# USTC-StarTeam/DR4SR

Measured on AMD Instinct MI355X. Metric: training sequences/sec, SASRec d=64 L=50, higher is better.
Workload: dtype f32; 1 GPU; SASRec on amazon-toys-shaped synthetic rows (BASELINE configs[1]): N=11925, L=50, d=64, 2 layers, 2 heads, FFN 128, dropout 0.50, B=256 rows/GPU/step, toys histogram (10.9% valid) seqlen; global_batch=256, seq_len=50, parallelism=dp1, hip_graph=True, steps_per_graph=30

## Files before the change

### dr4sr_amd/csrc/kernels.h

```cpp
#pragma once
#include <hip/hip_runtime.h>
#include <stdint.h>
#include "../../include/dr4sr_hip.h"
#include "../../include/dr4sr_hip_hooks.h"
#include "prep_body.h"

#define DR4SR_MAX_LAYERS 8

struct LayerWs {
    float* qkv;
    float* ctx;
    float* attn_st;
    unsigned* attn_keep;
    float* u1;
    float* y;
    float* st1;
    float* a;
    float* h;
    float* u2;
    float* st2;
    float* df;
    float* da;
    float* du1;
    float* dout;
// ... 73 lines not shown
    float* rd; int n_head;
    float* ln_part;
    const int* state; uint64_t seed; float p; float eps; int layer; int training;
    uint32_t sP, sA, sF;
    unsigned long long* stamps;
    const float* nx_in_w; const float* nx_in_b; float* nx_qkv;
    const float* up_dqkv; const float* up_in_w; const float* up_du1;
    const float* up_kv_part;
    TileAttnArgs at;
    int xcd;
    float* nx_dqkv_zero;
    float* dn_dqkv_zero;
    int wt_attn;
    unsigned short* row_keep;
    const unsigned short* sp;
};

struct EmbQkvArgs {
    const float* E; const float* P; const int64_t* idx; const int64_t* rows; const int* cu; const int* tile_seq; float* X;
    const float* W; const float* bias; float* QKV; const int* state;
    int B, L, n_items, training; uint64_t seed; float p;
    int* idx32;
    int2* tok; float* dqkv_zero;
    int xcd;
    int wf_layers;
    const unsigned short* sp;
    const float* inw;
};
struct QkvEmbBwdArgs {
    const float* dQKV; const float* W; const float* dU1; const int64_t* idx; const int64_t* rows; const int* cu; const int* tile_seq;
    float* dE; float* dP; const int* state; int B, L, n_items, training; uint64_t seed; float p;
    float* gout;
    const float* kv_part; const int2* tok;
    const unsigned short* sp;
    const float* inw; float* d_inw; const float* E; const float* P;
#ifdef DR4SR_EXPERIMENTS
    int xskip;
#endif
};

struct ScoreTileArgs {
    const float* E; float* dE; const int64_t* target; const int64_t* rows; const int* cu; const int* tile_seq; int64_t* neg_item; float* part;
    int sample_neg, n_items, B, L;
    int4* rec;
    int4* ent; unsigned char* off; const int* idx32; int logG;
    const float* phi; const float* gumbel; const int64_t* user_id; const unsigned long long* gate_in; unsigned long long* gate_out;
    float* w_out; float inv_tau; uint64_t meta_seed;
};

struct WgradJob {
    const float* G; int ldg; int gcol;
    const float* X; int ldx;
    float* dW; float* db;
    int ldw;
};
#define DR4SR_DET_MAX_SPLITS 320
#define DR4SR_WGRAD_MAX_JOBS 12
struct WgradArgs {
    WgradJob job[DR4SR_WGRAD_MAX_JOBS * DR4SR_MAX_LAYERS];
    int jobs_per_layer;
    const int* state; uint64_t seed; float p; int training;
    const float* ln_part; int64_t ln_layer_stride; float* grads; int64_t o_ln1_w; int64_t layer_stride;
    const float* score_part; float* tail; int B; int D;
    int score_tiles;
    int ln_tile_rows;
    int ln_rows[DR4SR_MAX_LAYERS];
    int qeb_plane;
    int layer0;
    int bf16x3;
    int xcd;
// ... 26 lines not shown
int carve_workspace(const dr4sr_sasrec_plan* p, Workspace* ws);

int launch_prep(const dr4sr_sasrec_plan* p, const Workspace& ws, int bump_rng, int zero_grads, hipStream_t s, int adam_bc = 0);
int make_prep_args(const dr4sr_sasrec_plan* p, const Workspace& ws, int bump_rng, PrepArgs* out);
int launch_embed_fwd(const dr4sr_sasrec_plan* p, const Workspace& ws, int training, hipStream_t s, const float* inw = nullptr);
int launch_embed_bwd(const dr4sr_sasrec_plan* p, const Workspace& ws, int training, hipStream_t s, const float* inw = nullptr, float* d_inw = nullptr);
int launch_unpack(const dr4sr_sasrec_plan* p, const Workspace& ws, const float* X, float* out, int mode, hipStream_t s);
int launch_pack(const dr4sr_sasrec_plan* p, const Workspace& ws, const float* dout, float* dX, int mode, hipStream_t s);

int launch_transpose_weights(const dr4sr_sasrec_plan* p, const Workspace& ws, hipStream_t s);
bool tile_bf3(const dr4sr_sasrec_plan* p, const Workspace& ws);
int launch_wsplit(const dr4sr_sasrec_plan* p, const Workspace& ws, hipStream_t s);
int launch_wfrag_write(const dr4sr_sasrec_plan* p, const Workspace& ws, hipStream_t s);
bool wfrag_img_on(const dr4sr_sasrec_plan* p, const Workspace& ws);
int launch_wsplit_raw(const float* params, unsigned short* img, int64_t o_in, int64_t o_out, int64_t o_w1, int64_t o_w2, int64_t layer_stride,
                      int E, int D, int F, int n_layer, hipStream_t s);
int launch_embqkv_fwd(const dr4sr_sasrec_plan* p, const Workspace& ws, int training, hipStream_t s, const float* inw = nullptr);
int launch_qkv_embed_bwd(const dr4sr_sasrec_plan* p, const Workspace& ws, int training, hipStream_t s, const float* inw = nullptr, float* d_inw = nullptr);
int launch_post_mid(const dr4sr_sasrec_plan* p, const Workspace& ws, int training, hipStream_t s, const dr4sr_meta_weighting* mw = nullptr);
int launch_qkv_fwd(const dr4sr_sasrec_plan* p, const Workspace& ws, int layer, hipStream_t s);
int launch_post_fwd(const dr4sr_sasrec_plan* p, const Workspace& ws, int layer, int training, hipStream_t s);
int launch_post_bwd(const dr4sr_sasrec_plan* p, const Workspace& ws, int layer, int training, hipStream_t s);
int launch_qkv_bwd(const dr4sr_sasrec_plan* p, const Workspace& ws, int layer, hipStream_t s);
int launch_wgrad(const dr4sr_sasrec_plan* p, const Workspace& ws, int training, int with_score, hipStream_t s, bool qeb = false,
                 bool meta = false, int l_lo = 0, int l_hi = -1, int table = -1, const float* inw = nullptr, float* d_inw = nullptr);
bool wgrad_table_jobs(const dr4sr_sasrec_plan* p, const Workspace& ws);
bool attn_in_tile(const dr4sr_sasrec_plan* p, const Workspace& ws);
bool attn_wave_on(const dr4sr_sasrec_plan* p, const Workspace& ws);
bool attn_fold_fwd(const dr4sr_sasrec_plan* p, const Workspace& ws);
PostArgs make_post_args(const dr4sr_sasrec_plan* p, const Workspace& ws, int layer, int training);
int launch_attn_tile_fwd(const dr4sr_sasrec_plan* p, const Workspace& ws, int layer, int training, hipStream_t s);
int launch_attn_tile_bwd(const dr4sr_sasrec_plan* p, const Workspace& ws, int layer, int training, hipStream_t s);
bool qeb_in_wgrad(const Workspace& ws);

int launch_attn_fwd(const dr4sr_sasrec_plan* p, const Workspace& ws, int layer, int training, hipStream_t s);
int launch_attn_bwd(const dr4sr_sasrec_plan* p, const Workspace& ws, int layer, int training, hipStream_t s);

struct GruWaveArgs {
    const float* gi1; const float* whh[2]; const float* wih2; const int* cu;
    float* r[2]; float* z[2]; float* n[2]; float* ghn[2]; float* hprev[2]; float* hout[2];
    const float* dhout; float* dgi[2]; float* dgh[2];
};
int launch_prep_raw(const int64_t* seqlen, const int64_t* rows, int* cu, int* state, int B, int L, int bump_rng, float* zero,
                    int64_t zero_floats, hipStream_t s);
int launch_prep_raw_hints(const int64_t* seqlen, const int64_t* rows, int* cu, int* state, int B, int L, int bump_rng, float* zero,
                          int64_t zero_floats, int* tile_seq, const PermSel& sel, hipStream_t s);
int launch_embed_fwd_raw(const float* E, const float* P, const int64_t* idx, const int64_t* rows, const int* cu, float* X, int B,
                         int L, int D, int n_items, const int* state, uint64_t seed, float p, int training, hipStream_t s, const float* inw = nullptr);
int launch_embed_bwd_raw(const float* dX, const int64_t* idx, const int64_t* rows, const int* cu, float* dE, float* dP, int B, int L,
                         int D, int n_items, const int* state, uint64_t seed, float p, int training, hipStream_t s,
                         const float* inw = nullptr, float* d_inw = nullptr, const float* E = nullptr, const float* P = nullptr);
int launch_unpack_raw(const float* X, const int* cu, float* out, int B, int L, int D, int last, hipStream_t s);
int launch_pack_raw(const float* dout, const int* cu, float* dX, int B, int L, int D, int last, hipStream_t s);
int launch_score_packed_raw(const float* Z, const float* E, float* dE, float* dZ, const int64_t* target, const int64_t* rows,
                            const int* cu, int64_t* neg_item, int sample_neg, float* part, const int* state, uint64_t seed,
                            int n_items, int B, int L, int D, hipStream_t s, int4* rec = nullptr);

int launch_attn2_fwd(const dr4sr_sasrec_plan* p, const Workspace& ws, int layer, int training, hipStream_t s);
int launch_attn2_bwd(const dr4sr_sasrec_plan* p, const Workspace& ws, int layer, int training, hipStream_t s);

int launch_score_packed(const dr4sr_sasrec_plan* p, const Workspace& ws, hipStream_t s);
int launch_adam(const dr4sr_sasrec_plan* p, hipStream_t s, const PrepArgs* next = nullptr);
```

### dr4sr_amd/csrc/linear.hip

```cpp
#include "common.h"
#include "kernels.h"
#include <cstdlib>
#define STAMP(i) do { if (A.stamps && blockIdx.x == 0 && threadIdx.x == 0) A.stamps[i] = __builtin_amdgcn_s_memtime(); } while (0)

extern __shared__ __attribute__((aligned(16))) float smem[];

__global__ __launch_bounds__(256) void k_transpose(const float* __restrict__ params, float* __restrict__ wT,
                                                   int64_t o_in, int64_t o_out, int64_t o_w1, int64_t o_w2,
                                                   int64_t layer_stride, int64_t wT_stride, int D, int F) {
    const int m = blockIdx.y, layer = blockIdx.z;
    const float* src;
    float* dst = wT + layer * wT_stride;
    int R, C;
    if (m == 0) { src = params + o_in + layer * layer_stride; R = 3 * D; C = D; }
    else if (m == 1) { src = params + o_out + layer * layer_stride; R = D; C = D; dst += 3 * D * D; }
    else if (m == 2) { src = params + o_w1 + layer * layer_stride; R = F; C = D; dst += 4 * D * D; }
    else { src = params + o_w2 + layer * layer_stride; R = D; C = F; dst += 4 * D * D + D * F; }
    for (int i = blockIdx.x * 256 + threadIdx.x; i < R * C; i += gridDim.x * 256) {
        const int r = i / C, c = i % C;
        dst[c * R + r] = src[i];
    }
}

int launch_transpose_weights(const dr4sr_sasrec_plan* p, const Workspace& ws, hipStream_t s) {
// ... 216 lines not shown
                o = ld4(A.E + id * D + c);
                const float4 pe = ld4(A.P + (size_t)pos * D + c);
                o = make_float4(o.x + pe.x, o.y + pe.y, o.z + pe.z, o.w + pe.w);
                if constexpr (WGT) {
                    const float w = A.inw[(size_t)b * A.L + pos];
                    o.x *= w; o.y *= w; o.z *= w; o.w *= w;
                }
                if (dodrop) {
                    const float4 m = drop4(rk, DR4SR_SITE_EMB, ((uint64_t)b * A.L + pos) * D + c);
                    o.x *= m.x; o.y *= m.y; o.z *= m.z; o.w *= m.w;
                }
                st4(A.X + (size_t)t * D + c, o);
            }
            st4(As + r * LDA + c, o);
        }
    }
    lds_barrier();
    TileAcc<BM, N> acc;
    tile_zero(acc);
    if constexpr (PFE) tile_mma_frag<BM, D, N>(As, LDA, f_in, acc);
    else tile_gemm<D == 128 && BM == 32, BM, D, N>(As, LDA, A.W, D, false, A.sp, WSplitGeo<D, 128>::E, 0, acc);
    if constexpr (EPB) tile_to_global<BM, N>(acc, A.QKV, N, in_b, t0, T); else tile_to_global<BM, N>(acc, A.QKV, N, A.bias, t0, T);
    if (A.dqkv_zero) zero_kv_rows<BM, D>(A.dqkv_zero, t0, T);
}

int launch_embqkv_fwd(const dr4sr_sasrec_plan* p, const Workspace& ws, int training, hipStream_t s, const float* inw) {
    const int D = p->D, bm = tile_rows(ws);
    const size_t lds = sizeof(float) * bm * (D + 4);
    dim3 grid((ws.Tmax + bm - 1) / bm), blk(256);
    EmbQkvArgs A;
    A.E = p->params + ws.off[0]; A.P = p->params + ws.off[1]; A.idx = p->in_item_id; A.rows = p->rows; A.cu = ws.cu; A.tile_seq = ws.tile_seq; A.X = ws.X[0];
    A.W = p->params + poff(ws, 0, P_IN_W); A.bias = p->params + poff(ws, 0, P_IN_B); A.QKV = ws.layer[0].qkv; A.state = p->state;
    A.B = p->B; A.L = p->L; A.n_items = p->n_items; A.training = training; A.seed = p->seed; A.p = p->p_drop;
    A.idx32 = de_owner_mode(ws) ? ws.idx32 : nullptr;
    A.sp = wsplit_of(p, ws, 0); A.wf_layers = 0; A.inw = inw;
    if (wfrag_img_on(p, ws)) { A.sp = reinterpret_cast<const unsigned short*>(ws.wfrag); A.wf_layers = p->n_layer; }
    const bool in_tile = attn_in_tile(p, ws);
    A.tok = (in_tile || ws.attn_tile_sa || attn_wave_on(p, ws)) ? ws.tok : nullptr; A.dqkv_zero = in_tile ? ws.layer[0].dqkv : nullptr;
    A.xcd = tile_xcd_order(p, ws) ? 1 : 0;
    if (A.xcd) grid.x = xcd_grid((int)grid.x, bm);
    if (wave_tiles(p, ws)) return launch_wt_embqkv_fwd(A, ws.Tmax, s);
#define EQ(B_) do { if (inw) { if (D == 64) hipLaunchKernelGGL((k_embqkv_fwd<B_, 64, true>), grid, blk, lds, s, A); \
                                else hipLaunchKernelGGL((k_embqkv_fwd<B_, 128, true>), grid, blk, lds, s, A); } \
                    else if (D == 64) hipLaunchKernelGGL((k_embqkv_fwd<B_, 64>), grid, blk, lds, s, A); \
                    else hipLaunchKernelGGL((k_embqkv_fwd<B_, 128>), grid, blk, lds, s, A); } while (0)
    BM_DISPATCH(bm, EQ);
#undef EQ
    return DR4SR_LAUNCH_CHECK();
}


struct LnCarry { float4 v; float mean, rstd; uint32_t keep; };
template <int F>
struct RowCarry { LnCarry ln1, ln2; float4 a[F / 64]; uint32_t akeep; };
__host__ __device__ constexpr bool carry_vals(int CARRY) { return CARRY != 0; }
__host__ __device__ constexpr bool carry_bits(int CARRY) { return CARRY == 1 || CARRY == 3; }
__device__ __forceinline__ uint32_t keep_bits4(const float4& m) {
    return (m.x != 0.f ? 1u : 0u) | (m.y != 0.f ? 2u : 0u) | (m.z != 0.f ? 4u : 0u) | (m.w != 0.f ? 8u : 0u);
}
__device__ __forceinline__ float4 keep_factors4(const RngKey& k, uint32_t bits) {
    return make_float4((bits & 1u) ? k.scale : 0.f, (bits & 2u) ? k.scale : 0.f, (bits & 4u) ? k.scale : 0.f, (bits & 8u) ? k.scale : 0.f);
}

template <int BM, int D, bool RES_IN_LDS, bool COPY_LDS, bool CARRY = false, bool KPRE = false, bool NOST = false, bool GPRE = false>
__device__ __forceinline__ void ln_rowpass(const float* __restrict__ Cs, int ldc, const float* res, int ldres,
                                           const float* __restrict__ lnw, const float* __restrict__ lnb, float eps,
                                           float* __restrict__ U, float* __restrict__ OUT, float* __restrict__ ST,
// ... 1244 lines not shown
    tile_zero(acc);
    tile_mma_xw<BM, K, D>(As, LDA, WT, D, acc);
    tile_to_lds<BM, D>(acc, Cs, LDC, nullptr);
    lds_barrier();
    constexpr int C4 = D / 4;
    for (int i = threadIdx.x; i < BM * C4; i += 256) {
        const int row = i / C4, c = (i % C4) * 4;
        if (t0 + row < T) {
            const float4 v = ld4(Cs + row * LDC + c), r = ld4(dU1 + (size_t)(t0 + row) * D + c);
            st4(dXo + (size_t)(t0 + row) * D + c, make_float4(v.x + r.x, v.y + r.y, v.z + r.z, v.w + r.w));
        }
    }
}

int launch_qkv_bwd(const dr4sr_sasrec_plan* p, const Workspace& ws, int layer, hipStream_t s) {
    const int D = p->D, bm = tile_rows(ws);
    const size_t lds = sizeof(float) * bm * ((3 * D + 4) + (D + 4));
    dim3 grid((ws.Tmax + bm - 1) / bm), blk(256);
    const float* WT = p->params + poff(ws, layer, P_IN_W);
    const LayerWs& lw = ws.layer[layer];
#define QB(B_) do { if (D == 64) { big_lds(k_qkv_bwd<B_, 64>, lds); hipLaunchKernelGGL((k_qkv_bwd<B_, 64>), grid, blk, lds, s, lw.dqkv, WT, lw.du1, ws.dX[layer], p->state); } \
                    else { big_lds(k_qkv_bwd<B_, 128>, lds); hipLaunchKernelGGL((k_qkv_bwd<B_, 128>), grid, blk, lds, s, lw.dqkv, WT, lw.du1, ws.dX[layer], p->state); } } while (0)
    BM_DISPATCH(bm, QB);
#undef QB
    return DR4SR_LAUNCH_CHECK();
}


#ifdef DR4SR_EMB_ADDS_FLOAT4
constexpr bool EMB_ADD_ROWS = false;
#else
constexpr bool EMB_ADD_ROWS = true;
#endif
template <int BM, int D, bool DET = false, bool WGT = false>
__device__ __forceinline__ void qkv_embed_bwd_body(const QkvEmbBwdArgs& A, const int t0, const int T) {
    constexpr int K = 3 * D, LDA = K + 4, LDC = D + 4, LPT = D / 4, TPB = 256 / LPT;
    float* As = smem;
    float* Cs = As + BM * LDA;
    float* accP = Cs + BM * LDC;
    int* ids = reinterpret_cast<int*>(accP + A.L * D);
    constexpr bool PFQ = BM == 16 && D == 64;
    WFragC<PFQ ? K : 16, 64> f_in;
    if constexpr (PFQ) wfrag_load(f_in, A.W, D);
    for (int i = threadIdx.x; i < A.L * D; i += 256) accP[i] = 0.f;
    load_tile_bm<BM, K>(As, LDA, A.dQKV, K, t0, T);
    lds_barrier();
    if constexpr (BM == 16 && DET) {
        det_kv_rows<D>(As, LDA, const_cast<float*>(A.dQKV), A.kv_part, A.tok, t0, T);
        lds_barrier();
    }
    TileAcc<BM, D> acc;
    tile_zero(acc);
    if constexpr (PFQ) tile_mma_frag<BM, K, D>(As, LDA, f_in, acc);
    else tile_gemm<D == 128 && BM == 32, BM, K, D>(As, LDA, A.W, D, true, A.sp, WSplitGeo<D, 128>::E, 0, acc);
    tile_to_lds<BM, D>(acc, Cs, LDC, nullptr);
    lds_barrier();
    const int c = (threadIdx.x % LPT) * 4;
    const bool dodrop = A.training && A.p > 0.f;
    const RngKey rk = make_rng(A.seed, (uint32_t)A.state[DR4SR_STATE_RNGSTEP], A.p);
    const int bh = A.tile_seq[t0 >> 4];
#pragma unroll
    for (int r0 = 0; r0 < BM; r0 += TPB) {
        const int r = r0 + threadIdx.x / LPT, t = t0 + r;
        if (r < BM && t < T) {
            const int b = find_seq_from(A.cu, A.B, t, bh), pos = t - A.cu[b];
            const int64_t row = A.rows ? A.rows[b] : b;
            const float4 v = ld4(Cs + r * LDC + c), u = ld4(A.dU1 + (size_t)t * D + c);
            float4 g = make_float4(v.x + u.x, v.y + u.y, v.z + u.z, v.w + u.w);
            if (dodrop) {
                const float4 m = drop4(rk, DR4SR_SITE_EMB, ((uint64_t)b * A.L + pos) * D + c);
                g.x *= m.x; g.y *= m.y; g.z *= m.z; g.w *= m.w;
            }
            if constexpr (WGT) {
                if (A.d_inw) {
                    int64_t ic = A.idx[row * A.L + pos];
                    ic = ic < 0 ? 0 : (ic >= A.n_items ? A.n_items - 1 : ic);
                    const float4 e = ld4(A.E + ic * D + c), pe = ld4(A.P + (size_t)pos * D + c);
                    const float sum = lane_group_sum<LPT>((g.x * (e.x + pe.x) + g.y * (e.y + pe.y)) + (g.z * (e.z + pe.z) + g.w * (e.w + pe.w)));
                    if (c == 0) A.d_inw[(size_t)b * A.L + pos] = sum;
                }
                const float w = A.inw[(size_t)b * A.L + pos];
                g.x *= w; g.y *= w; g.z *= w; g.w *= w;
            }
            if (A.gout) { st4(A.gout + (size_t)t * D + c, g); continue; }
            float* a = accP + pos * D + c;
            atomicAdd(a, g.x); atomicAdd(a + 1, g.y); atomicAdd(a + 2, g.z); atomicAdd(a + 3, g.w);
            const int64_t id = A.idx[row * A.L + pos];
            st4(Cs + r * LDC + c, g);
            if (c == 0) ids[r] = (id > 0 && id < A.n_items) ? (int)id : 0;
        } else if (r < BM && c == 0 && !A.gout) ids[r] = 0;
    }
    if (A.gout) return;
    __syncthreads();
#pragma unroll
    for (int r0 = 0; r0 < BM; r0 += TPB) {
        const int r = r0 + threadIdx.x / LPT;
        const int id = r < BM ? ids[r] : 0;
        unsigned long long same = 0;
        if constexpr (BM <= LPT) {
            const int j = threadIdx.x % LPT;
            const unsigned long long bal = __ballot(j < BM && id > 0 && ids[j < BM ? j : 0] == id);
            same = (bal >> ((threadIdx.x & 63) / LPT * LPT)) & ((1ull << BM) - 1ull);
        } else if (id > 0) {
            for (int q = 0; q < BM; ++q) same |= (unsigned long long)(ids[q] == id) << q;
        }
        if (id > 0 && (same & ((1ull << r) - 1ull)) == 0) {
            if constexpr (!DET && BM == 16 && EMB_ADD_ROWS) {
                const int j = threadIdx.x % LPT;
                float gk[4];
#pragma unroll
                for (int k = 0; k < 4; ++k) gk[k] = Cs[r * LDC + LPT * k + j];
                for (same = r + 1 < 64 ? same >> (r + 1) : 0; same; same &= same - 1) {
                    const int q = r + __ffsll((long long)same);
#pragma unroll
                    for (int k = 0; k < 4; ++k) gk[k] += Cs[q * LDC + LPT * k + j];
                }
                float* d = A.dE + (size_t)id * D + j;
                if (!XSKIP_EMB(A)) {
#pragma unroll
                    for (int k = 0; k < 4; ++k) unsafeAtomicAdd(d + LPT * k, gk[k]);
                }
                continue;
            }
            float4 g = ld4(Cs + r * LDC + c);
            for (same = r + 1 < 64 ? same >> (r + 1) : 0; same; same &= same - 1) {
                const int q = r + __ffsll((long long)same);
                const float4 o = ld4(Cs + q * LDC + c); g.x += o.x; g.y += o.y; g.z += o.z; g.w += o.w;
            }
            float* d = A.dE + (size_t)id * D + c;
            if (!XSKIP_EMB(A)) { unsafeAtomicAdd(d, g.x); unsafeAtomicAdd(d + 1, g.y); unsafeAtomicAdd(d + 2, g.z); unsafeAtomicAdd(d + 3, g.w); }
        }
    }
    for (int i = threadIdx.x; i < A.L * D; i += 256) {
        const float v = accP[i];
        if (v != 0.f) unsafeAtomicAdd(A.dP + i, v);
    }
}
template <int BM, int D, bool DET = false, bool WGT = false>
__global__ __launch_bounds__(256) void k_qkv_embed_bwd(const QkvEmbBwdArgs A) {
    const int T = A.state[DR4SR_STATE_T], t0 = blockIdx.x * BM;
    if (t0 >= T) return;
    qkv_embed_bwd_body<BM, D, DET, WGT>(A, t0, T);
}

static QkvEmbBwdArgs make_qeb_args(const dr4sr_sasrec_plan* p, const Workspace& ws, int training, const float* inw = nullptr, float* d_inw = nullptr) {
    const LayerWs& lw = ws.layer[0];
    QkvEmbBwdArgs A;
    A.dQKV = lw.dqkv; A.W = p->params + poff(ws, 0, P_IN_W); A.dU1 = lw.du1; A.idx = p->in_item_id; A.rows = p->rows; A.cu = ws.cu; A.tile_seq = ws.tile_seq;
    A.dE = p->grads + ws.off[0]; A.dP = p->grads + ws.off[1]; A.state = p->state; A.B = p->B; A.L = p->L; A.n_items = p->n_items;
    A.training = training; A.seed = p->seed; A.p = p->p_drop;
    A.gout = scatter_in_wgrad(ws) ? ws.dX[0] : nullptr;
    A.kv_part = (ws.det_lat && ws.det_kv && attn_in_tile(p, ws)) ? ws.det_kv : nullptr; A.tok = ws.tok;
    A.sp = wsplit_of(p, ws, 0);
    A.inw = inw; A.d_inw = inw ? d_inw : nullptr; A.E = p->params + ws.off[0]; A.P = p->params + ws.off[1];
#ifdef DR4SR_EXPERIMENTS
    A.xskip = DR4SR_XENV("DR4SR_ROWADDS_SKIP") ? (atoi(DR4SR_XENV("DR4SR_ROWADDS_SKIP")) & 4) : 0;
#endif
    return A;
}
bool qeb_in_wgrad(const Workspace& ws) {
    const bool off = DR4SR_ENV("DR4SR_QEB_SEPARATE") != nullptr || DR4SR_ENV("DR4SR_NO_FUSE") != nullptr;
    return !off && tile_rows(ws) == 16 && !ws.det_lat;
}

int launch_qkv_embed_bwd(const dr4sr_sasrec_plan* p, const Workspace& ws, int training, hipStream_t s, const float* inw, float* d_inw) {
    const int D = p->D, bm = tile_rows(ws);
    const size_t lds = sizeof(float) * (bm * ((3 * D + 4) + (D + 4)) + (size_t)p->L * D + bm);
    dim3 grid((ws.Tmax + bm - 1) / bm), blk(256);
    const QkvEmbBwdArgs A = make_qeb_args(p, ws, training, inw, d_inw);
    if (wave_tiles(p, ws) && wt_bwd_on() && A.gout) return launch_wt_qkv_embed_bwd(A, ws.Tmax, s);
#define QEW(B_, D_, DET_) do { big_lds((k_qkv_embed_bwd<B_, D_, DET_, true>), lds); hipLaunchKernelGGL((k_qkv_embed_bwd<B_, D_, DET_, true>), grid, blk, lds, s, A); } while (0)
#define QE(B_) do { if (A.inw) { if (B_ == 16 && A.kv_part) { if (D == 64) QEW(16, 64, true); else QEW(16, 128, true); } \
                                 else if (D == 64) QEW(B_, 64, false); else QEW(B_, 128, false); } \
                    else if (B_ == 16 && A.kv_part) { if (D == 64) { big_lds((k_qkv_embed_bwd<16, 64, true>), lds); hipLaunchKernelGGL((k_qkv_embed_bwd<16, 64, true>), grid, blk, lds, s, A); } \
                                                 else { big_lds((k_qkv_embed_bwd<16, 128, true>), lds); hipLaunchKernelGGL((k_qkv_embed_bwd<16, 128, true>), grid, blk, lds, s, A); } } \
                    else if (D == 64) { big_lds(k_qkv_embed_bwd<B_, 64>, lds); hipLaunchKernelGGL((k_qkv_embed_bwd<B_, 64>), grid, blk, lds, s, A); } \
                    else { big_lds(k_qkv_embed_bwd<B_, 128>, lds); hipLaunchKernelGGL((k_qkv_embed_bwd<B_, 128>), grid, blk, lds, s, A); } } while (0)
    BM_DISPATCH(bm, QE);
#undef QE
#undef QEW
    return DR4SR_LAUNCH_CHECK();
}


#ifdef DR4SR_EXPERIMENTS
#define WGRAD_ADD(P_, V_) do { if (!noadd) unsafeAtomicAdd(P_, V_); } while (0)
#else
#define WGRAD_ADD(P_, V_) unsafeAtomicAdd(P_, V_)
#endif

template <int NG, int KX>
__device__ __forceinline__ void wgrad_body(const WgradJob& J, const WgradArgs& A, float* __restrict__ part = nullptr, const int noadd = 0) {
    constexpr int NT = NG / 32, KT = KX / 32, TPW = (NT * KT) / 4;
    static_assert((NT * KT) % 4 == 0, "tile count must split over 4 waves");
    const int T = A.state[DR4SR_STATE_T];
// ... 379 lines not shown
        qn = 0;
    };
    constexpr int CH = 4;
    for (int base = ia; base < ib; base += 64 * CH) {
        int lo[CH], hi[CH];
#pragma unroll
        for (int k = 0; k < CH; ++k) {
            const int i = base + 64 * k + lane;
            lo[k] = 0; hi[k] = 0;
            if (i < ib) { const unsigned char* o = A.ow_off + (size_t)i * OS + owner; lo[k] = o[0]; hi[k] = o[1]; }
        }
#pragma unroll
        for (int k = 0; k < CH; ++k) {
            unsigned long long m = __ballot(hi[k] > lo[k]);
            while (m) {
                const int L = __ffsll((long long)m) - 1; m &= m - 1;
                const int tile = base + 64 * k + L, e0 = __builtin_amdgcn_readlane(lo[k], L), e1 = __builtin_amdgcn_readlane(hi[k], L);
                for (int e = e0; e < e1; ++e) {
                    if (lane == qn) pend = A.ow_ent[(size_t)tile * E + e];
                    if (++qn == QN) flush();
                }
            }
        }
    }
    flush();
    __syncthreads();
    for (int i = threadIdx.x; i < rpo * D; i += 256) {
        const float sum = (smem[i] + smem[(size_t)rpo * D + i]) + (smem[(size_t)2 * rpo * D + i] + smem[(size_t)3 * rpo * D + i]);
        const int id = ((i / D) << A.ow_logG) | owner;
        if (sum != 0.f && id < A.sc_n_items) A.sc_dE[(size_t)id * D + (i % D)] += sum;
    }
}

template <int D, int F, bool BF, bool SUB = false, bool BLK = false, int TB = 0, bool WGT = false>
__device__ __forceinline__ void wgrad_kernel_body(const WgradArgs& A, const QkvEmbBwdArgs& Q, const int noadd = 0) {
    const int layer = A.layer0 + (A.qeb_plane ? (int)blockIdx.z - 1 : (int)blockIdx.z);
    if (!SUB && layer < A.layer0) {
        const int T = A.state[DR4SR_STATE_T], nblk = gridDim.x * gridDim.y;
        for (int tile = blockIdx.y * gridDim.x + blockIdx.x; tile * 16 < T; tile += nblk) {
            qkv_embed_bwd_body<16, D, false, WGT>(Q, tile * 16, T);
            __syncthreads();
        }
        return;
    }
    int j = (int)blockIdx.y;
    if constexpr (!BLK) {
        const bool tz = (int)blockIdx.z == A.qeb_plane;
        if (A.ow_on && (int)blockIdx.y < A.ow_planes) {
            if (tz) { if (A.ow_ent) owner_job_sorted<D>(A, blockIdx.y * gridDim.x + blockIdx.x); else owner_job<D>(A, blockIdx.y * gridDim.x + blockIdx.x); }
            return;
        }
        j = (int)blockIdx.y - (A.ow_on ? A.ow_planes : 0) - (A.sc_g ? 1 : 0);
        if (j < 0) { if (tz) scatter_job<D>(A); return; }
    }
    if constexpr (BLK && TB > 0) {
        constexpr int RB = 32 * TB, NDD = (D / RB) * (D / 32), NFD = (F / RB) * (D / 32), NB = 4 * NDD + NFD + (D / RB) * (F / 32);
        if (j == NB) { reduce_jobs(A, layer); return; }
        const int jj = j < 4 * NDD ? j / NDD : (j < 4 * NDD + NFD ? 4 : 5), q = j - (jj < 5 ? jj * NDD : 4 * NDD + NFD);
        const int ncb = (jj == 5 ? F : D) / 32, rb = q / ncb, cb = q % ncb;
        WgradJob Jb = A.job[layer * A.jobs_per_layer + jj];
        const int ldw = Jb.ldw ? Jb.ldw : (jj == 5 ? F : D);
        Jb.gcol += RB * rb; Jb.X += 32 * cb; Jb.dW += (size_t)RB * rb * ldw + 32 * cb; Jb.ldw = ldw;
        Jb.db = (Jb.db && cb == 0) ? Jb.db + RB * rb : nullptr;
        wgrad_ksplit_body<TB>(Jb, A, noadd);
        return;
    } else if constexpr (BLK) {
        constexpr int RD = D / 64, RF = F / 64, NDD = RD * RD, NB = 4 * NDD + 2 * RD * RF;
        if (j == NB) { reduce_jobs(A, layer); return; }
        int jj, rb, cb;
        if (j < 4 * NDD) { jj = j / NDD; rb = (j % NDD) / RD; cb = (j % NDD) % RD; }
        else if (j < 4 * NDD + RF * RD) { jj = 4; rb = (j - 4 * NDD) / RD; cb = (j - 4 * NDD) % RD; }
        else { jj = 5; rb = (j - 4 * NDD - RF * RD) / RF; cb = (j - 4 * NDD - RF * RD) % RF; }
        WgradJob Jb = A.job[layer * A.jobs_per_layer + jj];
        const int ldw = Jb.ldw ? Jb.ldw : (jj == 5 ? F : D);
        Jb.gcol += 64 * rb; Jb.X += 64 * cb; Jb.dW += (size_t)64 * rb * ldw + 64 * cb; Jb.ldw = ldw;
        Jb.db = (Jb.db && cb == 0) ? Jb.db + 64 * rb : nullptr;
        wgrad_body<64, 64>(Jb, A, nullptr, noadd);
        return;
    }
    if (j == A.jobs_per_layer) { reduce_jobs(A, layer); return; }
    const WgradJob& J = A.job[layer * A.jobs_per_layer + j];
    float* part = A.det ? A.det + ((size_t)(layer * A.jobs_per_layer + j) * gridDim.x + blockIdx.x) * A.det_stride : nullptr;
    if constexpr (SUB) {
        wgrad_body_bf<64, 64>(J, A.state, part);
    } else if constexpr (BF) {
        if (j < 4) wgrad_body_bf<D, D>(J, A.state, part);
        else if (j == 4) wgrad_body_bf<F, D>(J, A.state, part);
        else wgrad_body_bf<D, F>(J, A.state, part);
    } else {
        if (j < 4) wgrad_body<D, D>(J, A, part);
        else if (j == 4) wgrad_body<F, D>(J, A, part);
        else wgrad_body<D, F>(J, A, part);
    }
}
template <int D, int F, bool WGT = false>
__global__ __launch_bounds__(256) void k_wgrad(const WgradArgs A, const QkvEmbBwdArgs Q) { wgrad_kernel_body<D, F, false, false, false, 0, WGT>(A, Q); }
template <int D, int F, bool WGT = false>
__global__ __launch_bounds__(256) void k_wgrad_bf(const WgradArgs A, const QkvEmbBwdArgs Q) { wgrad_kernel_body<D, F, true, false, false, 0, WGT>(A, Q); }
template <int D, int F>
__global__ __launch_bounds__(256) void k_wgrad_bf64(const WgradArgs A, const QkvEmbBwdArgs Q) { wgrad_kernel_body<D, F, true, true>(A, Q); }
template <int D, int F, int TB = 0, bool WGT = false>
__global__ __launch_bounds__(256) void k_wgrad_blk(const WgradArgs A, const QkvEmbBwdArgs Q, const int noadd) {
    wgrad_kernel_body<D, F, false, false, true, TB, WGT>(A, Q, noadd);
}


struct DetDims { short ng[DR4SR_WGRAD_MAX_JOBS], kx[DR4SR_WGRAD_MAX_JOBS]; };
__global__ __launch_bounds__(256) void k_wgrad_det_reduce(const WgradArgs A, const DetDims dm, const int gw, const int gemm, const int table,
                                                          const int ln_cols) {
    const int layer = A.layer0 + (int)blockIdx.z, j = blockIdx.y, T = A.state[DR4SR_STATE_T];
    const int e = blockIdx.x * 256 + threadIdx.x;
    if (j < A.jobs_per_layer) {
        if (!gemm) return;
        const WgradJob& J = A.job[layer * A.jobs_per_layer + j];
        const int NG = dm.ng[j], KX = dm.kx[j], nsplit = min(gw, (T + 63) / 64);
        if (e >= NG * KX + NG) return;
        const float* p = A.det + (size_t)(layer * A.jobs_per_layer + j) * gw * A.det_stride + e;
        if (e >= NG * KX && !J.db) return;
        const float s = det_sum(p, nsplit, (size_t)A.det_stride);
        if (e < NG * KX) J.dW[(size_t)(e / KX) * (J.ldw ? J.ldw : KX) + e % KX] += s;
        else J.db[e - NG * KX] += s;
    } else if (j == A.jobs_per_layer) {
        if (!gemm || e >= ln_cols) return;
        const float* p = A.det_ln + (size_t)layer * gw * 4 * A.D + e;
        const float s = det_sum(p, gw, (size_t)4 * A.D);
        A.grads[A.o_ln1_w + (size_t)layer * A.layer_stride + e] += s;
    } else {
        if (!table || blockIdx.z != 0 || !A.det_dp || e >= A.sc_L * A.D) return;
        A.sc_dP[e] += det_sum(A.det_dp + e, gw, (size_t)A.sc_L * A.D);
    }
}

__device__ __forceinline__ void reduce_jobs_fmlp(const WgradArgs& A) {
    const int T = A.state[DR4SR_STATE_T], ntiles = (T + A.ln_tile_rows - 1) / A.ln_tile_rows, D = A.D, layer = blockIdx.z;
    const float* part = A.ln_part + (size_t)layer * A.ln_layer_stride;
    float* g = A.grads + A.o_ln1_w + (size_t)layer * A.layer_stride;
// ... 197 lines not shown
    const bool wq = A.qeb_plane && Q.inw;
    size_t lds = sub64 ? wgrad_lds_base(p) : sizeof(float) * 64 * (D + F > 2 * D ? D + F : 2 * D);
    if (scatter && sizeof(float) * p->L * D > lds) lds = sizeof(float) * p->L * D;
    A.det = nullptr; A.det_ln = nullptr; A.det_dp = nullptr; A.det_stride = 0;
    if (ws.det && ws.det_part && ws.scale_wg && !blk_env_on()) {
        A.det = ws.det_part; A.det_stride = (int)ws.det_stride; A.det_ln = ws.det_ln; A.det_dp = (scatter && de_owner_mode(ws)) ? ws.det_dp : nullptr;
        A.xcd = 0;
    }
    A.ow_ent = nullptr; A.ow_off = nullptr;
    A.ow_on = 0; A.ow_rec = nullptr; A.ow_idx32 = nullptr; A.ow_z = nullptr; A.ow_logG = 0; A.ow_planes = 0; A.ow_rpo = 0;
    if (scatter && de_owner_mode(ws)) {
        const int logG = owner_logG(p);
        A.ow_on = 1; A.ow_logG = logG; A.ow_rpo = (p->n_items + (1 << logG) - 1) >> logG; A.ow_planes = ((1 << logG) + gw - 1) / gw;
        A.ow_rec = with_score == 2 ? ws.de_rec : nullptr; A.ow_idx32 = ws.idx32; A.ow_z = ws.X[p->n_layer];
        if (with_score == 2 && owner_sorted(p, ws, meta)) { A.ow_ent = ws.de_ent; A.ow_off = ws.de_off; }
    }
    const char* blk_env = DR4SR_XENV("DR4SR_WGRAD_BLK");
    const bool blk64 = !A.bf16x3 && !scatter && (blk_env ? atoi(blk_env) != 0 : !ws.scale);
    const char* ks_env = DR4SR_XENV("DR4SR_WGRAD_KSPLIT");
    const int ks = !blk64 ? 0 : ks_env ? atoi(ks_env) : 2;
    if (ks < 0 || ks > 2) return DR4SR_E_ARG;
    if (ks) gw = gw_env && gw_max > 0 ? gw_max : 8;
    const int NY = ks ? (4 * D * D + 2 * D * F) / (1024 * ks) : blk64 ? 4 * (D / 64) * (D / 64) + 2 * (D / 64) * (F / 64) : NJ;
    if (blk64 && !scatter) lds = sizeof(float) * 64 * 128;
    const int noadd = DR4SR_XENV("DR4SR_WGRAD_NOADD") ? atoi(DR4SR_XENV("DR4SR_WGRAD_NOADD")) : 0;
    if (A.det) {
        if (blk64 || gw > DR4SR_DET_MAX_SPLITS) return DR4SR_E_SHAPE;
        for (int jj = 0; jj < NJ; ++jj) {
            const int ng = sub64 ? 64 : (jj == 4 ? F : D), kx = sub64 ? 64 : (jj == 5 ? F : D);
            if (ng * kx + ng > A.det_stride) return DR4SR_E_SHAPE;
        }
    }
    dim3 grid(gw, (gemm ? NY + 1 : 0) + (scatter ? 1 : 0) + A.ow_planes, (gemm ? l_hi - l_lo : 1) + A.qeb_plane), blk(256);
    const size_t lds_q = sizeof(float) * (16 * ((3 * D + 4) + (D + 4)) + (size_t)p->L * D + 16);
    if (A.qeb_plane && lds_q > lds) lds = lds_q;
#define WGB(D_, F_, TB_) do { big_lds((k_wgrad_blk<D_, F_, TB_>), lds); hipLaunchKernelGGL((k_wgrad_blk<D_, F_, TB_>), grid, blk, lds, s, A, Q, noadd); } while (0)
#ifdef DR4SR_EXPERIMENTS
#define WGX(D_, F_) if (blk64 && ks == 0) WGB(D_, F_, 0); else if (ks == 1) WGB(D_, F_, 1); else
#else
#define WGX(D_, F_)
#endif
#define WGW(K_) do { big_lds((K_), lds); hipLaunchKernelGGL((K_), grid, blk, lds, s, A, Q); } while (0)
#define WG(D_, F_) do { if (wq) { if (blk64 && ks == 2) { big_lds((k_wgrad_blk<D_, F_, 2, true>), lds); hipLaunchKernelGGL((k_wgrad_blk<D_, F_, 2, true>), grid, blk, lds, s, A, Q, noadd); } \
                                  else if (blk64 || sub64) return DR4SR_E_SHAPE;       \
                                  else if (A.bf16x3) WGW((k_wgrad_bf<D_, F_, true>)); else WGW((k_wgrad<D_, F_, true>)); } \
                        else WGX(D_, F_) if (blk64) WGB(D_, F_, 2); \
                        else if (sub64) { big_lds(k_wgrad_bf64<D_, F_>, lds); hipLaunchKernelGGL((k_wgrad_bf64<D_, F_>), grid, blk, lds, s, A, Q); } \
                        else if (A.bf16x3) { big_lds(k_wgrad_bf<D_, F_>, lds); hipLaunchKernelGGL((k_wgrad_bf<D_, F_>), grid, blk, lds, s, A, Q); } \
                        else { big_lds(k_wgrad<D_, F_>, lds); hipLaunchKernelGGL((k_wgrad<D_, F_>), grid, blk, lds, s, A, Q); } } while (0)
    if (D == 64 && F == 128) WG(64, 128);
    else if (D == 128 && F == 128) WG(128, 128);
    else if (D == 64 && F == 256) WG(64, 256);
    else return DR4SR_E_SHAPE;
#undef WG
#undef WGW
#undef WGX
#undef WGB
    if (A.det) {
        DetDims dm;
        for (int jj = 0; jj < NJ; ++jj) {
            if (sub64) { dm.ng[jj] = 64; dm.kx[jj] = 64; }
            else { dm.ng[jj] = (short)(jj == 4 ? F : D); dm.kx[jj] = (short)(jj == 5 ? F : D); }
        }
        int maxe = 4 * D > p->L * D ? 4 * D : p->L * D;
        for (int jj = 0; jj < NJ; ++jj) {
            if (dm.ng[jj] * dm.kx[jj] + dm.ng[jj] > maxe) maxe = dm.ng[jj] * dm.kx[jj] + dm.ng[jj];
        }
        hipLaunchKernelGGL(k_wgrad_det_reduce, dim3((maxe + 255) / 256, NJ + 2, gemm ? l_hi - l_lo : 1), dim3(256), 0, s, A, dm, gw, gemm ? 1 : 0,
                           scatter ? 1 : 0, 4 * D);
    }
    return DR4SR_LAUNCH_CHECK();
}
```

Baseline: 3.090 million sequences/s.

## Prefetch per-row embedding-backward inputs early and bound dP flush in fused qkv-embed bwd

Adds an ENT variant of the fused qkv/embedding backward body, used when the wgrad kernel hosts the qeb plane at d=64. It loads the token map, 32-bit item ids, dU1 rows and dropout keep bits into registers up front, overlapping them with the dQKV tile load. It also replaces the per-row sequence search and the int64 index gather with precomputed tok/idx32 lookups. The dP flush is limited to positions actually touched by the tile, at the cost of more register pressure and a small amount of extra LDS.

```diff
diff --git a/dr4sr_amd/csrc/kernels.h b/dr4sr_amd/csrc/kernels.h
--- a/dr4sr_amd/csrc/kernels.h
+++ b/dr4sr_amd/csrc/kernels.h
@@ -129,10 +129,13 @@
     float* dE; float* dP; const int* state; int B, L, n_items, training; uint64_t seed; float p;
     float* gout;
     const float* kv_part; const int2* tok;
+    const int* idx32;
     const unsigned short* sp;
     const float* inw; float* d_inw; const float* E; const float* P;
 #ifdef DR4SR_EXPERIMENTS
     int xskip;
+    unsigned long long* stamps;
+    int stamp_t0;
 #endif
 };
 
@@ -225,6 +228,7 @@
 int launch_attn_tile_fwd(const dr4sr_sasrec_plan* p, const Workspace& ws, int layer, int training, hipStream_t s);
 int launch_attn_tile_bwd(const dr4sr_sasrec_plan* p, const Workspace& ws, int layer, int training, hipStream_t s);
 bool qeb_in_wgrad(const Workspace& ws);
+bool emb_entry_words(const dr4sr_sasrec_plan* p, const Workspace& ws);
 
 int launch_attn_fwd(const dr4sr_sasrec_plan* p, const Workspace& ws, int layer, int training, hipStream_t s);
 int launch_attn_bwd(const dr4sr_sasrec_plan* p, const Workspace& ws, int layer, int training, hipStream_t s);
diff --git a/dr4sr_amd/csrc/linear.hip b/dr4sr_amd/csrc/linear.hip
--- a/dr4sr_amd/csrc/linear.hip
+++ b/dr4sr_amd/csrc/linear.hip
@@ -272,7 +272,7 @@
     A.E = p->params + ws.off[0]; A.P = p->params + ws.off[1]; A.idx = p->in_item_id; A.rows = p->rows; A.cu = ws.cu; A.tile_seq = ws.tile_seq; A.X = ws.X[0];
     A.W = p->params + poff(ws, 0, P_IN_W); A.bias = p->params + poff(ws, 0, P_IN_B); A.QKV = ws.layer[0].qkv; A.state = p->state;
     A.B = p->B; A.L = p->L; A.n_items = p->n_items; A.training = training; A.seed = p->seed; A.p = p->p_drop;
-    A.idx32 = de_owner_mode(ws) ? ws.idx32 : nullptr;
+    A.idx32 = (de_owner_mode(ws) || emb_entry_words(p, ws)) ? ws.idx32 : nullptr;
     A.sp = wsplit_of(p, ws, 0); A.wf_layers = 0; A.inw = inw;
     if (wfrag_img_on(p, ws)) { A.sp = reinterpret_cast<const unsigned short*>(ws.wfrag); A.wf_layers = p->n_layer; }
     const bool in_tile = attn_in_tile(p, ws);
@@ -1583,19 +1583,78 @@
 #else
 constexpr bool EMB_ADD_ROWS = true;
 #endif
-template <int BM, int D, bool DET = false, bool WGT = false>
+#ifdef DR4SR_EXPERIMENTS
+#define QSTAMP(i) do { if (A.stamps && t0 == A.stamp_t0 && threadIdx.x == 0) A.stamps[i] = __builtin_amdgcn_s_memtime(); } while (0)
+#else
+#define QSTAMP(i) do { } while (0)
+#endif
+template <int BM, int D, bool DET = false, bool WGT = false, bool ENT = false>
 __device__ __forceinline__ void qkv_embed_bwd_body(const QkvEmbBwdArgs& A, const int t0, const int T) {
     constexpr int K = 3 * D, LDA = K + 4, LDC = D + 4, LPT = D / 4, TPB = 256 / LPT;
+    QSTAMP(32);
     float* As = smem;
     float* Cs = As + BM * LDA;
     float* accP = Cs + BM * LDC;
     int* ids = reinterpret_cast<int*>(accP + A.L * D);
+    static_assert(!ENT || (BM == 16 && !DET && D == 64), "entry words: the 16-row latency form at d = 64");
+    constexpr int NR = ENT ? BM / TPB : 1, NT = ENT ? BM * (K / 4) / 256 : 1;
+    int* poss = ids + BM;
+    int2 e_tok[NR]; int e_id[NR]; float4 e_du[NR]; uint32_t e_keep[NR];
+    float e_w[NR]; float4 e_ev[NR], e_pv[NR];
+    RngKey e_rk;
+    if constexpr (ENT) {
+        const int ce = (threadIdx.x % LPT) * 4;
+#pragma unroll
+        for (int k = 0; k < NR; ++k) {
+            const int t = t0 + k * TPB + threadIdx.x / LPT, tl = t < T ? t : T - 1;
+            e_tok[k] = A.tok[tl]; e_id[k] = A.idx32[tl]; e_du[k] = ld4(A.dU1 + (size_t)tl * D + ce);
+        }
+        e_rk = make_rng(A.seed, (uint32_t)A.state[DR4SR_STATE_RNGSTEP], A.p);
+    }
     constexpr bool PFQ = BM == 16 && D == 64;
     WFragC<PFQ ? K : 16, 64> f_in;
     if constexpr (PFQ) wfrag_load(f_in, A.W, D);
     for (int i = threadIdx.x; i < A.L * D; i += 256) accP[i] = 0.f;
-    load_tile_bm<BM, K>(As, LDA, A.dQKV, K, t0, T);
-    lds_barrier();
+    if constexpr (ENT) {
+        constexpr int C4 = K / 4;
+        float4 tv[NT];
+#pragma unroll
+        for (int j = 0; j < NT; ++j) {
+            const int i = threadIdx.x + 256 * j, row = i / C4, cc = (i % C4) * 4;
+            tv[j] = t0 + row < T ? ld4(A.dQKV + (size_t)(t0 + row) * K + cc) : make_float4(0.f, 0.f, 0.f, 0.f);
+        }
+        if (A.training && A.p > 0.f) {
+            const int ce = (threadIdx.x % LPT) * 4;
+#pragma unroll
+            for (int k = 0; k < NR; ++k) {
+                const int t = t0 + k * TPB + threadIdx.x / LPT, tl = t < T ? t : T - 1;
+                const int b = min(e_tok[k].y & 0xfffff, A.B - 1), pos = min(max(tl - e_tok[k].x, 0), A.L - 1);
+                e_keep[k] = keep_bits4(drop4(e_rk, DR4SR_SITE_EMB, ((uint64_t)b * A.L + pos) * D + ce));
+            }
+        }
+        __builtin_amdgcn_sched_barrier(0);
+#pragma unroll
+        for (int j = 0; j < NT; ++j) {
+            const int i = threadIdx.x + 256 * j, row = i / C4, cc = (i % C4) * 4;
+            st4(As + row * LDA + cc, tv[j]);
+        }
+    } else load_tile_bm<BM, K>(As, LDA, A.dQKV, K, t0, T);
+    lds_barrier(); QSTAMP(33);
+    if constexpr (ENT && WGT) {
+        const int ce = (threadIdx.x % LPT) * 4;
+#pragma unroll
+        for (int k = 0; k < NR; ++k) {
+            const int t = t0 + k * TPB + threadIdx.x / LPT, tl = t < T ? t : T - 1;
+            const int b = min(e_tok[k].y & 0xfffff, A.B - 1), pos = min(max(tl - e_tok[k].x, 0), A.L - 1);
+            e_w[k] = A.inw[(size_t)b * A.L + pos];
+            if (A.d_inw) {
+                const int64_t row = A.rows ? A.rows[b] : b;
+                int64_t ic = A.idx[row * A.L + pos];
+                ic = ic < 0 ? 0 : (ic >= A.n_items ? A.n_items - 1 : ic);
+                e_ev[k] = ld4(A.E + ic * D + ce); e_pv[k] = ld4(A.P + (size_t)pos * D + ce);
+            }
+        }
+    }
     if constexpr (BM == 16 && DET) {
         det_kv_rows<D>(As, LDA, const_cast<float*>(A.dQKV), A.kv_part, A.tok, t0, T);
         lds_barrier();
@@ -1605,44 +1664,74 @@
     if constexpr (PFQ) tile_mma_frag<BM, K, D>(As, LDA, f_in, acc);
     else tile_gemm<D == 128 && BM == 32, BM, K, D>(As, LDA, A.W, D, true, A.sp, WSplitGeo<D, 128>::E, 0, acc);
     tile_to_lds<BM, D>(acc, Cs, LDC, nullptr);
-    lds_barrier();
+    lds_barrier(); QSTAMP(34);
     const int c = (threadIdx.x % LPT) * 4;
     const bool dodrop = A.training && A.p > 0.f;
-    const RngKey rk = make_rng(A.seed, (uint32_t)A.state[DR4SR_STATE_RNGSTEP], A.p);
-    const int bh = A.tile_seq[t0 >> 4];
-#pragma unroll
-    for (int r0 = 0; r0 < BM; r0 += TPB) {
-        const int r = r0 + threadIdx.x / LPT, t = t0 + r;
-        if (r < BM && t < T) {
-            const int b = find_seq_from(A.cu, A.B, t, bh), pos = t - A.cu[b];
-            const int64_t row = A.rows ? A.rows[b] : b;
-            const float4 v = ld4(Cs + r * LDC + c), u = ld4(A.dU1 + (size_t)t * D + c);
-            float4 g = make_float4(v.x + u.x, v.y + u.y, v.z + u.z, v.w + u.w);
-            if (dodrop) {
-                const float4 m = drop4(rk, DR4SR_SITE_EMB, ((uint64_t)b * A.L + pos) * D + c);
-                g.x *= m.x; g.y *= m.y; g.z *= m.z; g.w *= m.w;
-            }
-            if constexpr (WGT) {
-                if (A.d_inw) {
-                    int64_t ic = A.idx[row * A.L + pos];
-                    ic = ic < 0 ? 0 : (ic >= A.n_items ? A.n_items - 1 : ic);
-                    const float4 e = ld4(A.E + ic * D + c), pe = ld4(A.P + (size_t)pos * D + c);
-                    const float sum = lane_group_sum<LPT>((g.x * (e.x + pe.x) + g.y * (e.y + pe.y)) + (g.z * (e.z + pe.z) + g.w * (e.w + pe.w)));
-                    if (c == 0) A.d_inw[(size_t)b * A.L + pos] = sum;
+    if constexpr (ENT) {
+#pragma unroll
+        for (int k = 0; k < NR; ++k) {
+            const int r = k * TPB + threadIdx.x / LPT, t = t0 + r;
+            if (t < T) {
+                const int b = min(e_tok[k].y & 0xfffff, A.B - 1), pos = min(max(t - e_tok[k].x, 0), A.L - 1);
+                const float4 v = ld4(Cs + r * LDC + c), u = e_du[k];
+                float4 g = make_float4(v.x + u.x, v.y + u.y, v.z + u.z, v.w + u.w);
+                if (dodrop) {
+                    const float4 m = keep_factors4(e_rk, e_keep[k]);
+                    g.x *= m.x; g.y *= m.y; g.z *= m.z; g.w *= m.w;
                 }
-                const float w = A.inw[(size_t)b * A.L + pos];
-                g.x *= w; g.y *= w; g.z *= w; g.w *= w;
-            }
-            if (A.gout) { st4(A.gout + (size_t)t * D + c, g); continue; }
-            float* a = accP + pos * D + c;
-            atomicAdd(a, g.x); atomicAdd(a + 1, g.y); atomicAdd(a + 2, g.z); atomicAdd(a + 3, g.w);
-            const int64_t id = A.idx[row * A.L + pos];
-            st4(Cs + r * LDC + c, g);
-            if (c == 0) ids[r] = (id > 0 && id < A.n_items) ? (int)id : 0;
-        } else if (r < BM && c == 0 && !A.gout) ids[r] = 0;
+                if constexpr (WGT) {
+                    if (A.d_inw) {
+                        const float4 e = e_ev[k], pe = e_pv[k];
+                        const float sum = lane_group_sum<LPT>((g.x * (e.x + pe.x) + g.y * (e.y + pe.y)) + (g.z * (e.z + pe.z) + g.w * (e.w + pe.w)));
+                        if (c == 0) A.d_inw[(size_t)b * A.L + pos] = sum;
+                    }
+                    const float w = e_w[k];
+                    g.x *= w; g.y *= w; g.z *= w; g.w *= w;
+                }
+                float* a = accP + pos * D + c;
+                atomicAdd(a, g.x); atomicAdd(a + 1, g.y); atomicAdd(a + 2, g.z); atomicAdd(a + 3, g.w);
+                st4(Cs + r * LDC + c, g);
+                if (c == 0) { ids[r] = (unsigned)e_id[k] < (unsigned)A.n_items ? e_id[k] : 0; poss[r] = pos; }
+            } else if (c == 0) { ids[r] = 0; poss[r] = -1; }
+        }
+    } else {
+        const RngKey rk = make_rng(A.seed, (uint32_t)A.state[DR4SR_STATE_RNGSTEP], A.p);
+        const int bh = A.tile_seq[t0 >> 4];
+#pragma unroll
+        for (int r0 = 0; r0 < BM; r0 += TPB) {
+            const int r = r0 + threadIdx.x / LPT, t = t0 + r;
+            if (r < BM && t < T) {
+                const int b = find_seq_from(A.cu, A.B, t, bh), pos = t - A.cu[b];
+                const int64_t row = A.rows ? A.rows[b] : b;
+                const float4 v = ld4(Cs + r * LDC + c), u = ld4(A.dU1 + (size_t)t * D + c);
+                float4 g = make_float4(v.x + u.x, v.y + u.y, v.z + u.z, v.w + u.w);
+                if (dodrop) {
+                    const float4 m = drop4(rk, DR4SR_SITE_EMB, ((uint64_t)b * A.L + pos) * D + c);
+                    g.x *= m.x; g.y *= m.y; g.z *= m.z; g.w *= m.w;
+                }
+                if constexpr (WGT) {
+                    if (A.d_inw) {
+                        int64_t ic = A.idx[row * A.L + pos];
+                        ic = ic < 0 ? 0 : (ic >= A.n_items ? A.n_items - 1 : ic);
+                        const float4 e = ld4(A.E + ic * D + c), pe = ld4(A.P + (size_t)pos * D + c);
+                        const float sum = lane_group_sum<LPT>((g.x * (e.x + pe.x) + g.y * (e.y + pe.y)) + (g.z * (e.z + pe.z) + g.w * (e.w + pe.w)));
+                        if (c == 0) A.d_inw[(size_t)b * A.L + pos] = sum;
+                    }
+                    const float w = A.inw[(size_t)b * A.L + pos];
+                    g.x *= w; g.y *= w; g.z *= w; g.w *= w;
+                }
+                if (A.gout) { st4(A.gout + (size_t)t * D + c, g); continue; }
+                float* a = accP + pos * D + c;
+                atomicAdd(a, g.x); atomicAdd(a + 1, g.y); atomicAdd(a + 2, g.z); atomicAdd(a + 3, g.w);
+                const int64_t id = A.idx[row * A.L + pos];
+                st4(Cs + r * LDC + c, g);
+                if (c == 0) ids[r] = (id > 0 && id < A.n_items) ? (int)id : 0;
+            } else if (r < BM && c == 0 && !A.gout) ids[r] = 0;
+        }
     }
     if (A.gout) return;
-    __syncthreads();
+    if constexpr (ENT) lds_barrier(); else __syncthreads();
+    QSTAMP(35);
 #pragma unroll
     for (int r0 = 0; r0 < BM; r0 += TPB) {
         const int r = r0 + threadIdx.x / LPT;
@@ -1682,10 +1771,19 @@
             if (!XSKIP_EMB(A)) { unsafeAtomicAdd(d, g.x); unsafeAtomicAdd(d + 1, g.y); unsafeAtomicAdd(d + 2, g.z); unsafeAtomicAdd(d + 3, g.w); }
         }
     }
-    for (int i = threadIdx.x; i < A.L * D; i += 256) {
+    QSTAMP(36);
+    int nflush = A.L * D;
+    if constexpr (ENT) {
+        int pmax = 0;
+#pragma unroll
+        for (int q = 0; q < BM; ++q) pmax = poss[q] > pmax ? poss[q] : pmax;
+        nflush = (pmax + 1) * D;
+    }
+    for (int i = threadIdx.x; i < nflush; i += 256) {
         const float v = accP[i];
         if (v != 0.f) unsafeAtomicAdd(A.dP + i, v);
     }
+    QSTAMP(37);
 }
 template <int BM, int D, bool DET = false, bool WGT = false>
 __global__ __launch_bounds__(256) void k_qkv_embed_bwd(const QkvEmbBwdArgs A) {
@@ -1701,17 +1799,26 @@
     A.dE = p->grads + ws.off[0]; A.dP = p->grads + ws.off[1]; A.state = p->state; A.B = p->B; A.L = p->L; A.n_items = p->n_items;
     A.training = training; A.seed = p->seed; A.p = p->p_drop;
     A.gout = scatter_in_wgrad(ws) ? ws.dX[0] : nullptr;
-    A.kv_part = (ws.det_lat && ws.det_kv && attn_in_tile(p, ws)) ? ws.det_kv : nullptr; A.tok = ws.tok;
+    A.kv_part = (ws.det_lat && ws.det_kv && attn_in_tile(p, ws)) ? ws.det_kv : nullptr; A.tok = ws.tok; A.idx32 = ws.idx32;
     A.sp = wsplit_of(p, ws, 0);
     A.inw = inw; A.d_inw = inw ? d_inw : nullptr; A.E = p->params + ws.off[0]; A.P = p->params + ws.off[1];
 #ifdef DR4SR_EXPERIMENTS
     A.xskip = DR4SR_XENV("DR4SR_ROWADDS_SKIP") ? (atoi(DR4SR_XENV("DR4SR_ROWADDS_SKIP")) & 4) : 0;
+    A.stamps = DR4SR_XENV("DR4SR_STAMPS") ? reinterpret_cast<unsigned long long*>(ws.dctx) : nullptr;
+    A.stamp_t0 = 16 * (DR4SR_XENV("DR4SR_QEB_STAMP_TILE") ? atoi(DR4SR_XENV("DR4SR_QEB_STAMP_TILE")) : 0);
 #endif
     return A;
 }
 bool qeb_in_wgrad(const Workspace& ws) {
     const bool off = DR4SR_ENV("DR4SR_QEB_SEPARATE") != nullptr || DR4SR_ENV("DR4SR_NO_FUSE") != nullptr;
     return !off && tile_rows(ws) == 16 && !ws.det_lat;
+}
+bool emb_entry_words(const dr4sr_sasrec_plan* p, const Workspace& ws) {
+#ifdef DR4SR_NO_EMB_ENTRY
+    return false;
+#else
+    return p->D == 64 && qeb_in_wgrad(ws) && !scatter_in_wgrad(ws) && (attn_in_tile(p, ws) || ws.attn_tile_sa || attn_wave_on(p, ws));
+#endif
 }
 
 int launch_qkv_embed_bwd(const dr4sr_sasrec_plan* p, const Workspace& ws, int training, hipStream_t s, const float* inw, float* d_inw) {
@@ -2157,13 +2264,13 @@
     }
 }
 
-template <int D, int F, bool BF, bool SUB = false, bool BLK = false, int TB = 0, bool WGT = false>
+template <int D, int F, bool BF, bool SUB = false, bool BLK = false, int TB = 0, bool WGT = false, bool ENT = false>
 __device__ __forceinline__ void wgrad_kernel_body(const WgradArgs& A, const QkvEmbBwdArgs& Q, const int noadd = 0) {
     const int layer = A.layer0 + (A.qeb_plane ? (int)blockIdx.z - 1 : (int)blockIdx.z);
     if (!SUB && layer < A.layer0) {
         const int T = A.state[DR4SR_STATE_T], nblk = gridDim.x * gridDim.y;
         for (int tile = blockIdx.y * gridDim.x + blockIdx.x; tile * 16 < T; tile += nblk) {
-            qkv_embed_bwd_body<16, D, false, WGT>(Q, tile * 16, T);
+            qkv_embed_bwd_body<16, D, false, WGT, ENT>(Q, tile * 16, T);
             __syncthreads();
         }
         return;
@@ -2224,9 +2331,9 @@
 __global__ __launch_bounds__(256) void k_wgrad_bf(const WgradArgs A, const QkvEmbBwdArgs Q) { wgrad_kernel_body<D, F, true, false, false, 0, WGT>(A, Q); }
 template <int D, int F>
 __global__ __launch_bounds__(256) void k_wgrad_bf64(const WgradArgs A, const QkvEmbBwdArgs Q) { wgrad_kernel_body<D, F, true, true>(A, Q); }
-template <int D, int F, int TB = 0, bool WGT = false>
+template <int D, int F, int TB = 0, bool WGT = false, bool ENT = false>
 __global__ __launch_bounds__(256) void k_wgrad_blk(const WgradArgs A, const QkvEmbBwdArgs Q, const int noadd) {
-    wgrad_kernel_body<D, F, false, false, true, TB, WGT>(A, Q, noadd);
+    wgrad_kernel_body<D, F, false, false, true, TB, WGT, ENT>(A, Q, noadd);
 }
 
 
@@ -2490,9 +2597,11 @@
         }
     }
     dim3 grid(gw, (gemm ? NY + 1 : 0) + (scatter ? 1 : 0) + A.ow_planes, (gemm ? l_hi - l_lo : 1) + A.qeb_plane), blk(256);
-    const size_t lds_q = sizeof(float) * (16 * ((3 * D + 4) + (D + 4)) + (size_t)p->L * D + 16);
+    const bool ent = A.qeb_plane && blk64 && ks == 2 && !Q.gout && emb_entry_words(p, ws);
+    const size_t lds_q = sizeof(float) * (16 * ((3 * D + 4) + (D + 4)) + (size_t)p->L * D + 16 + (ent ? 16 : 0));
     if (A.qeb_plane && lds_q > lds) lds = lds_q;
 #define WGB(D_, F_, TB_) do { big_lds((k_wgrad_blk<D_, F_, TB_>), lds); hipLaunchKernelGGL((k_wgrad_blk<D_, F_, TB_>), grid, blk, lds, s, A, Q, noadd); } while (0)
+#define WGE(D_, F_, W_) do { big_lds((k_wgrad_blk<D_, F_, 2, W_, true>), lds); hipLaunchKernelGGL((k_wgrad_blk<D_, F_, 2, W_, true>), grid, blk, lds, s, A, Q, noadd); } while (0)
 #ifdef DR4SR_EXPERIMENTS
 #define WGX(D_, F_) if (blk64 && ks == 0) WGB(D_, F_, 0); else if (ks == 1) WGB(D_, F_, 1); else
 #else
@@ -2506,7 +2615,9 @@
                         else if (sub64) { big_lds(k_wgrad_bf64<D_, F_>, lds); hipLaunchKernelGGL((k_wgrad_bf64<D_, F_>), grid, blk, lds, s, A, Q); } \
                         else if (A.bf16x3) { big_lds(k_wgrad_bf<D_, F_>, lds); hipLaunchKernelGGL((k_wgrad_bf<D_, F_>), grid, blk, lds, s, A, Q); } \
                         else { big_lds(k_wgrad<D_, F_>, lds); hipLaunchKernelGGL((k_wgrad<D_, F_>), grid, blk, lds, s, A, Q); } } while (0)
-    if (D == 64 && F == 128) WG(64, 128);
+    if (ent && F == 128) { if (wq) WGE(64, 128, true); else WGE(64, 128, false); }
+    else if (ent && F == 256) { if (wq) WGE(64, 256, true); else WGE(64, 256, false); }
+    else if (D == 64 && F == 128) WG(64, 128);
     else if (D == 128 && F == 128) WG(128, 128);
     else if (D == 64 && F == 256) WG(64, 256);
     else return DR4SR_E_SHAPE;
@@ -2514,6 +2625,7 @@
 #undef WGW
 #undef WGX
 #undef WGB
+#undef WGE
     if (A.det) {
         DetDims dm;
         for (int jj = 0; jj < NJ; ++jj) {
```

After: 3.102 million sequences/s (median of 6 runs). Within noise of the previous version (+0.4%).
